# microsoft/KubeGPU

Measured on AMD Instinct MI355X. Metric: scheduled_set_allreduce_busbw_GBps, higher is better.
Workload: dtype uint8; 1 GPU; model=rccl-xgmi-allreduce-probe, global_batch=2000, seq_len=1073741824, parallelism=allreduce-ring-1gpu, mode=hbm_d2d_copy, curve_point=k1-degenerate-hbm, buffer_bytes=1073741824, scenario=BASELINE.json k=1, rank_pinning=ROCR_VISIBLE_DEVICES, pinned_device=0, pinned_bdf=0000:75:00.0, bdf_verified=True

## Files before the change

### kubegpu_amd/csrc/gpuprobe.hip

```cpp

#include <torch/extension.h>
#include <ATen/hip/HIPContext.h>
#include <ATen/hip/impl/HIPGuardImplMasqueradingAsCUDA.h>
#include <hip/hip_runtime.h>

#include <cstdint>

#define WAVE 64
#define BLOCK 256
#define DEFAULT_COPY_BLOCKS 1024
#define DEFAULT_WRITE_BLOCKS 640

__global__ void copy_kernel_v4(const uint4* __restrict__ src,
                               uint4* __restrict__ dst, size_t n4) {
  size_t i = (size_t)blockIdx.x * blockDim.x + threadIdx.x;
  size_t stride = (size_t)gridDim.x * blockDim.x;
  for (; i < n4; i += stride) dst[i] = src[i];
}

typedef unsigned int uint4v __attribute__((ext_vector_type(4)));

__global__ void copy_kernel_v4_nt(const uint4v* __restrict__ src,
                                  uint4v* __restrict__ dst, size_t n4) {
  size_t i = (size_t)blockIdx.x * blockDim.x + threadIdx.x;
  size_t stride = (size_t)gridDim.x * blockDim.x;
  for (; i < n4; i += stride) {
    uint4v v = __builtin_nontemporal_load(&src[i]);
    __builtin_nontemporal_store(v, &dst[i]);
  }
}

__global__ void copy_kernel_v4_nt_u4(const uint4v* __restrict__ src,
                                     uint4v* __restrict__ dst, size_t n4) {
  size_t tid = (size_t)blockIdx.x * blockDim.x + threadIdx.x;
  size_t stride = (size_t)gridDim.x * blockDim.x;
  size_t i = tid;
  size_t bound = n4 >= 3 * stride ? n4 - 3 * stride : 0;
  for (; i < bound; i += 4 * stride) {
    uint4v a = __builtin_nontemporal_load(&src[i]);
    uint4v b = __builtin_nontemporal_load(&src[i + stride]);
    uint4v c = __builtin_nontemporal_load(&src[i + 2 * stride]);
    uint4v d = __builtin_nontemporal_load(&src[i + 3 * stride]);
    __builtin_nontemporal_store(a, &dst[i]);
    __builtin_nontemporal_store(b, &dst[i + stride]);
    __builtin_nontemporal_store(c, &dst[i + 2 * stride]);
    __builtin_nontemporal_store(d, &dst[i + 3 * stride]);
  }
  for (; i < n4; i += stride) {
    uint4v v = __builtin_nontemporal_load(&src[i]);
    __builtin_nontemporal_store(v, &dst[i]);
  }
}

__global__ void copy_kernel_v4_nt_chunk(const uint4v* __restrict__ src,
                                        uint4v* __restrict__ dst, size_t n4) {
  size_t per_block = (n4 + gridDim.x - 1) / gridDim.x;
  size_t begin = (size_t)blockIdx.x * per_block;
  size_t end = begin + per_block < n4 ? begin + per_block : n4;
  for (size_t i = begin + threadIdx.x; i < end; i += blockDim.x) {
    uint4v v = __builtin_nontemporal_load(&src[i]);
    __builtin_nontemporal_store(v, &dst[i]);
  }
}

__global__ void copy_kernel_v4_mixed(const uint4v* __restrict__ src,
                                     uint4v* __restrict__ dst, size_t n4) {
  size_t i = (size_t)blockIdx.x * blockDim.x + threadIdx.x;
  size_t stride = (size_t)gridDim.x * blockDim.x;
  for (; i < n4; i += stride) {
    uint4v v = src[i];
    __builtin_nontemporal_store(v, &dst[i]);
  }
}

__global__ void copy_kernel_b(const unsigned char* __restrict__ src,
                              unsigned char* __restrict__ dst, size_t n) {
  size_t i = (size_t)blockIdx.x * blockDim.x + threadIdx.x;
  size_t stride = (size_t)gridDim.x * blockDim.x;
  for (; i < n; i += stride) dst[i] = src[i];
}

__global__ void read_sum_kernel(const uint4* __restrict__ src, size_t n4,
                                unsigned long long* __restrict__ out) {
  size_t i = (size_t)blockIdx.x * blockDim.x + threadIdx.x;
  size_t stride = (size_t)gridDim.x * blockDim.x;
  unsigned long long acc = 0;
  for (; i < n4; i += stride) {
    uint4 v = src[i];
    acc += (unsigned long long)v.x + v.y + v.z + v.w;
  }
  __shared__ unsigned long long sh[BLOCK / WAVE];
  for (int off = WAVE / 2; off > 0; off >>= 1)
    acc += __shfl_down(acc, off, WAVE);
  int lane = threadIdx.x % WAVE;
  int wid = threadIdx.x / WAVE;
  if (lane == 0) sh[wid] = acc;
  __syncthreads();
  if (threadIdx.x == 0) {
    unsigned long long total = 0;
    for (int w = 0; w < BLOCK / WAVE; ++w) total += sh[w];
    atomicAdd(out, total);
  }
}

__global__ void fill_kernel_v4_nt(uint4v* __restrict__ dst, size_t n4,
                                  unsigned int word) {
  uint4v v = {word, word, word, word};
  size_t i = (size_t)blockIdx.x * blockDim.x + threadIdx.x;
  size_t stride = (size_t)gridDim.x * blockDim.x;
  for (; i < n4; i += stride) __builtin_nontemporal_store(v, &dst[i]);
}


#define MAX_BLOCKS (1 << 20)

static void check_buf(const at::Tensor& t) {
  TORCH_CHECK(t.is_cuda(), "gpuprobe: tensors must be on GPU");
  TORCH_CHECK(t.is_contiguous(), "gpuprobe: tensors must be contiguous");
}

static size_t check_vec_buf(const at::Tensor& t) {
  check_buf(t);
  TORCH_CHECK(t.nbytes() > 0 && t.nbytes() % 16 == 0,
              "gpuprobe: nbytes must be a positive multiple of 16, got ", t.nbytes());
  TORCH_CHECK((uintptr_t)t.data_ptr() % 16 == 0,
              "gpuprobe: tensor storage must be 16-byte aligned");
  return t.nbytes() / 16;
}

static void check_pair(const at::Tensor& dst, const at::Tensor& src) {
  check_buf(dst);
  check_buf(src);
  TORCH_CHECK(src.nbytes() == dst.nbytes(), "gpuprobe: size mismatch");
  TORCH_CHECK(src.device() == dst.device(),
              "gpuprobe: tensors must be on the same device");
  uintptr_t s = (uintptr_t)src.data_ptr(), d = (uintptr_t)dst.data_ptr();
  size_t n = src.nbytes();
  TORCH_CHECK(s == d || s + n <= d || d + n <= s,
              "gpuprobe: dst and src overlap in part");
}

static int check_threads(int64_t threads_arg) {
  TORCH_CHECK(threads_arg >= 0 && threads_arg % WAVE == 0 && threads_arg <= 1024,
              "threads: multiple of 64, <=1024");
  return threads_arg > 0 ? (int)threads_arg : BLOCK;
}

static int pick_blocks(int64_t blocks_arg, size_t n4, int threads, int dflt) {
  TORCH_CHECK(blocks_arg >= 0 && blocks_arg <= MAX_BLOCKS,
              "gpuprobe: blocks out of range 0..", MAX_BLOCKS);
  if (blocks_arg > 0) return (int)blocks_arg;
  return (int)std::min<size_t>((n4 + threads - 1) / threads, (size_t)dflt);
}

static void check_variant(int64_t variant) {
  TORCH_CHECK(variant >= 0 && variant <= 3, "gpuprobe: variant ", variant,
              " out of range 0..3");
}

static void launch_copy(const void* src, void* dst, size_t n4, int64_t variant,
                        bool nontemporal, int blocks, int threads,
                        hipStream_t stream) {
  if (variant == 1)
    hipLaunchKernelGGL(copy_kernel_v4_nt_u4, dim3(blocks), dim3(threads), 0, stream,
                       (const uint4v*)src, (uint4v*)dst, n4);
  else if (variant == 2)
    hipLaunchKernelGGL(copy_kernel_v4_nt_chunk, dim3(blocks), dim3(threads), 0,
                       stream, (const uint4v*)src, (uint4v*)dst, n4);
  else if (variant == 3)
    hipLaunchKernelGGL(copy_kernel_v4_mixed, dim3(blocks), dim3(threads), 0,
                       stream, (const uint4v*)src, (uint4v*)dst, n4);
  else if (nontemporal)
    hipLaunchKernelGGL(copy_kernel_v4_nt, dim3(blocks), dim3(threads), 0, stream,
                       (const uint4v*)src, (uint4v*)dst, n4);
  else
    hipLaunchKernelGGL(copy_kernel_v4, dim3(blocks), dim3(threads), 0, stream,
                       (const uint4*)src, (uint4*)dst, n4);
}

static void launch_read_sum(const void* src, size_t n4, void* out, int blocks,
                            hipStream_t stream) {
  hipLaunchKernelGGL(read_sum_kernel, dim3(blocks), dim3(BLOCK), 0, stream,
                     (const uint4*)src, n4, (unsigned long long*)out);
}

static void launch_fill(void* dst, size_t n4, unsigned int word, int blocks,
                        hipStream_t stream) {
  hipLaunchKernelGGL(fill_kernel_v4_nt, dim3(blocks), dim3(BLOCK), 0, stream,
                     (uint4v*)dst, n4, word);
}

void copy(at::Tensor dst, at::Tensor src) {
  check_pair(dst, src);
  size_t nbytes = src.nbytes();
  if (nbytes == 0) return;
  const at::hip::OptionalHIPGuardMasqueradingAsCUDA guard(at::device_of(dst));
  auto stream = at::hip::getCurrentHIPStream();
  if ((((uintptr_t)src.data_ptr() | (uintptr_t)dst.data_ptr() | nbytes) & 15) == 0) {
    size_t n4 = nbytes / 16;
    int blocks = (int)std::min<size_t>((n4 + BLOCK - 1) / BLOCK, DEFAULT_COPY_BLOCKS);
    launch_copy(src.data_ptr(), dst.data_ptr(), n4, 0, true, blocks, BLOCK, stream);
  } else {
    int blocks = (int)std::min<size_t>((nbytes + BLOCK - 1) / BLOCK, 4096);
    hipLaunchKernelGGL(copy_kernel_b, dim3(blocks), dim3(BLOCK), 0, stream,
                       (const unsigned char*)src.data_ptr(),
                       (unsigned char*)dst.data_ptr(), nbytes);
  }
  C10_HIP_KERNEL_LAUNCH_CHECK();
}

void copy_variant(at::Tensor dst, at::Tensor src, int64_t variant, bool nontemporal,
                  int64_t blocks_arg, int64_t threads_arg) {
  check_pair(dst, src);
  size_t n4 = check_vec_buf(src);
  check_vec_buf(dst);
  check_variant(variant);
  int threads = check_threads(threads_arg);
  int blocks = pick_blocks(blocks_arg, n4, threads, DEFAULT_COPY_BLOCKS);
  const at::hip::OptionalHIPGuardMasqueradingAsCUDA guard(at::device_of(dst));
  auto stream = at::hip::getCurrentHIPStream();
  launch_copy(src.data_ptr(), dst.data_ptr(), n4, variant, nontemporal, blocks,
              threads, stream);
  C10_HIP_KERNEL_LAUNCH_CHECK();
}

uint64_t read_sum(at::Tensor src, int64_t blocks_arg) {
  size_t n4 = check_vec_buf(src);
  int blocks = pick_blocks(blocks_arg, n4, BLOCK, DEFAULT_COPY_BLOCKS);
  const at::hip::OptionalHIPGuardMasqueradingAsCUDA guard(at::device_of(src));
  at::Tensor out = at::zeros({1}, src.options().dtype(at::kLong));
  auto stream = at::hip::getCurrentHIPStream();
  launch_read_sum(src.data_ptr(), n4, out.data_ptr(), blocks, stream);
  C10_HIP_KERNEL_LAUNCH_CHECK();
  C10_HIP_CHECK(hipStreamSynchronize(stream));
  return (uint64_t)out.item<int64_t>();
}

void fill_word(at::Tensor dst, int64_t word, int64_t blocks_arg) {
  size_t n4 = check_vec_buf(dst);
  TORCH_CHECK(word >= 0 && word <= 0xFFFFFFFFLL, "gpuprobe: word must be a u32");
  int blocks = pick_blocks(blocks_arg, n4, BLOCK, DEFAULT_WRITE_BLOCKS);
  const at::hip::OptionalHIPGuardMasqueradingAsCUDA guard(at::device_of(dst));
  auto stream = at::hip::getCurrentHIPStream();
  launch_fill(dst.data_ptr(), n4, (unsigned int)word, blocks, stream);
  C10_HIP_KERNEL_LAUNCH_CHECK();
}

static void check_timed_args(int64_t nbytes, int64_t iters) {
  TORCH_CHECK(nbytes > 0 && nbytes % 16 == 0, "nbytes must be positive, 16-aligned");
  TORCH_CHECK(iters >= 1, "iters must be at least 1");
}

#define POISON 0xA5

template <typename Launch>
static float timed_ms(hipStream_t stream, int64_t iters, Launch&& launch) {
  for (int w = 0; w < 3; ++w) launch();
  hipEvent_t t0, t1;
  (void)hipEventCreate(&t0);
  (void)hipEventCreate(&t1);
  (void)hipEventRecord(t0, stream);
  for (int64_t i = 0; i < iters; ++i) launch();
  (void)hipEventRecord(t1, stream);
  (void)hipEventSynchronize(t1);
  float ms = 0.f;
  (void)hipEventElapsedTime(&ms, t0, t1);
  (void)hipEventDestroy(t0);
  (void)hipEventDestroy(t1);
  C10_HIP_KERNEL_LAUNCH_CHECK();
  return ms;
}

double copy_bw_gbps(int64_t nbytes, int64_t iters, int64_t blocks_arg,
                    bool nontemporal, int64_t variant, int64_t threads_arg) {
  check_timed_args(nbytes, iters);
  check_variant(variant);
  size_t n4 = (size_t)nbytes / 16;
  int threads = check_threads(threads_arg);
  int blocks = pick_blocks(blocks_arg, n4, threads, DEFAULT_COPY_BLOCKS);
  auto opts = at::TensorOptions().dtype(at::kByte).device(at::kCUDA);
  at::Tensor src = at::empty({nbytes}, opts);
  at::Tensor dst = at::empty({nbytes}, opts);
  src.fill_(1);
  dst.fill_(POISON);
  auto stream = at::hip::getCurrentHIPStream();
  float ms = timed_ms(stream, iters, [&]() {
    launch_copy(src.data_ptr(), dst.data_ptr(), n4, variant, nontemporal, blocks,
                threads, stream);
  });
  TORCH_CHECK(at::equal(dst, src), "copy_bw_gbps: variant ", variant,
              " produced wrong output");
  double sec = ms / 1e3;
  return (double)nbytes * 2.0 * iters / sec / 1e9;
}

double write_bw_gbps(int64_t nbytes, int64_t iters, int64_t blocks_arg) {
  check_timed_args(nbytes, iters);
  size_t n4 = (size_t)nbytes / 16;
  int blocks = pick_blocks(blocks_arg, n4, BLOCK, DEFAULT_WRITE_BLOCKS);
  auto opts = at::TensorOptions().dtype(at::kByte).device(at::kCUDA);
  at::Tensor dst = at::empty({nbytes}, opts);
  dst.fill_(POISON);
  auto stream = at::hip::getCurrentHIPStream();
  float ms = timed_ms(stream, iters, [&]() {
    launch_fill(dst.data_ptr(), n4, 0x01010101u, blocks, stream);
  });
  TORCH_CHECK(dst.min().item<uint8_t>() == 1 && dst.max().item<uint8_t>() == 1,
              "write_bw_gbps: fill produced wrong output");
  return (double)nbytes * iters / (ms / 1e3) / 1e9;
}

double read_bw_gbps(int64_t nbytes, int64_t iters, int64_t blocks_arg) {
  check_timed_args(nbytes, iters);
  size_t n4 = (size_t)nbytes / 16;
  int blocks = pick_blocks(blocks_arg, n4, BLOCK, DEFAULT_COPY_BLOCKS);
  auto opts = at::TensorOptions().dtype(at::kByte).device(at::kCUDA);
  at::Tensor src = at::empty({nbytes}, opts);
  src.fill_(1);
  at::Tensor out = at::zeros({1}, at::TensorOptions().dtype(at::kLong).device(at::kCUDA));
  auto stream = at::hip::getCurrentHIPStream();
  float ms = timed_ms(stream, iters, [&]() {
    launch_read_sum(src.data_ptr(), n4, out.data_ptr(), blocks, stream);
  });
  uint64_t want = (uint64_t)(3 + iters) * ((uint64_t)nbytes / 4) * 0x01010101ULL;
  TORCH_CHECK((uint64_t)out.item<int64_t>() == want,
              "read_bw_gbps: read_sum_kernel produced a wrong sum");
  double sec = ms / 1e3;
  return (double)nbytes * iters / sec / 1e9;
}

void bind_memcheck(py::module_& m);
void bind_cucheck(py::module_& m);
void bind_mxcheck(py::module_& m);
void bind_fpcheck(py::module_& m);
void bind_atomcheck(py::module_& m);
void bind_lanecheck(py::module_& m);
void bind_hostlink(py::module_& m);

PYBIND11_MODULE(TORCH_EXTENSION_NAME, m) {
  bind_memcheck(m);
  bind_cucheck(m);
  bind_mxcheck(m);
  bind_fpcheck(m);
  bind_atomcheck(m);
  bind_lanecheck(m);
  bind_hostlink(m);
  m.def("copy", &copy, "streaming uint4 copy kernel (dst, src)",
        py::call_guard<py::gil_scoped_release>());
  m.def("copy_variant", &copy_variant,
        "one untimed launch of a copy_bw_gbps variant (dst, src)",
        py::call_guard<py::gil_scoped_release>(),
        py::arg("dst"), py::arg("src"), py::arg("variant") = 0,
        py::arg("nontemporal") = true, py::arg("blocks") = 0,
        py::arg("threads") = 0);
  m.def("read_sum", &read_sum, "u64 sum of all 32-bit words (one launch)",
        py::call_guard<py::gil_scoped_release>(),
        py::arg("src"), py::arg("blocks") = 0);
  m.def("fill_word", &fill_word, "NT fill of every 32-bit word (one launch)",
        py::call_guard<py::gil_scoped_release>(),
        py::arg("dst"), py::arg("word"), py::arg("blocks") = 0);
  m.def("copy_bw_gbps", &copy_bw_gbps, "timed d2d copy bandwidth",
        py::call_guard<py::gil_scoped_release>(),
        py::arg("nbytes"), py::arg("iters") = 20, py::arg("blocks") = 0,
        py::arg("nontemporal") = true, py::arg("variant") = 0,
        py::arg("threads") = 0);
  m.def("read_bw_gbps", &read_bw_gbps, "timed read bandwidth",
        py::call_guard<py::gil_scoped_release>(),
        py::arg("nbytes"), py::arg("iters") = 20, py::arg("blocks") = 0);
  m.def("write_bw_gbps", &write_bw_gbps, "timed write-only (NT fill) bandwidth",
        py::call_guard<py::gil_scoped_release>(),
        py::arg("nbytes"), py::arg("iters") = 20, py::arg("blocks") = 0);
}
```

### kubegpu_amd/probe/bandwidth.py

```python

from __future__ import annotations

import importlib
import os
import sys

_EXT_DIR = os.path.join(os.path.dirname(os.path.dirname(os.path.abspath(__file__))), "_ext")
_ext = None


class NativeExtensionMissing(RuntimeError):
    pass


def load_ext(required: bool = True):
    global _ext
    if _ext is not None:
        return _ext
    import torch

    if _EXT_DIR not in sys.path:
        sys.path.insert(0, _EXT_DIR)
    try:
        _ext = importlib.import_module("_gpuprobe")
    except ImportError as e:
        if required or torch.cuda.is_available():
            raise NativeExtensionMissing(
                "_gpuprobe HIP extension is not built; run "
                "`python -m kubegpu_amd.build_native` (gfx950) — refusing "
                f"to fall back to eager PyTorch on a GPU box: {e}"
            ) from e
        return None
    return _ext


def copy(dst, src) -> None:
    load_ext().copy(dst, src)


def copy_variant(
    dst,
    src,
    variant: int = 0,
    nontemporal: bool = True,
    blocks: int = 0,
    threads: int = 0,
) -> None:
    load_ext().copy_variant(dst, src, variant, nontemporal, blocks, threads)


def read_sum(src, blocks: int = 0) -> int:
    return load_ext().read_sum(src, blocks)


def fill_word(dst, word: int, blocks: int = 0) -> None:
    load_ext().fill_word(dst, word, blocks)


def d2d_copy_bw_gbps(
    nbytes: int = 1 << 30,
    iters: int = 20,
    blocks: int = 0,
    nontemporal: bool = True,
    variant: int = 0,
) -> float:
    return load_ext().copy_bw_gbps(nbytes, iters, blocks, nontemporal, variant)


def read_bw_gbps(nbytes: int = 1 << 30, iters: int = 20, blocks: int = 0) -> float:
    return load_ext().read_bw_gbps(nbytes, iters, blocks)


def write_bw_gbps(nbytes: int = 1 << 30, iters: int = 20, blocks: int = 0) -> float:
    return load_ext().write_bw_gbps(nbytes, iters, blocks)
```

Before: 5825 GB/s.

## Route aligned copy through unrolled tile kernel with LDS-limited occupancy

Adds a templated tile copy kernel where each block copies contiguous tiles of BLOCK*U vectors with nontemporal loads and stores issued in batches. Occupancy is capped by requesting dummy dynamic LDS so that only a few blocks (three by default) stay resident per CU, and the grid is sized up to MAX_BLOCKS. The default copy() path now uses unroll 2 and residency 3 in place of the grid-stride NT kernel with 1024 blocks. This aims to make DRAM access more address-ordered and cut contention, but fewer resident waves may fail to hide memory latency.

```diff
diff --git a/kubegpu_amd/csrc/gpuprobe.hip b/kubegpu_amd/csrc/gpuprobe.hip
--- a/kubegpu_amd/csrc/gpuprobe.hip
+++ b/kubegpu_amd/csrc/gpuprobe.hip
@@ -4,11 +4,15 @@
 #include <ATen/hip/impl/HIPGuardImplMasqueradingAsCUDA.h>
 #include <hip/hip_runtime.h>
 
+#include <atomic>
 #include <cstdint>
+#include <string>
 
 #define WAVE 64
 #define BLOCK 256
 #define DEFAULT_COPY_BLOCKS 1024
+#define COPY_TILES_UNROLL 2
+#define COPY_TILES_RESIDENT 3
 #define DEFAULT_WRITE_BLOCKS 640
 
 __global__ void copy_kernel_v4(const uint4* __restrict__ src,
@@ -70,6 +74,34 @@
   for (; i < n4; i += stride) {
     uint4v v = src[i];
     __builtin_nontemporal_store(v, &dst[i]);
+  }
+}
+
+template <int U>
+__global__ void __launch_bounds__(BLOCK)
+copy_kernel_tiles(const uint4v* __restrict__ src, uint4v* __restrict__ dst, size_t n4) {
+  constexpr size_t T = (size_t)BLOCK * U;
+  const size_t tiles = (n4 + T - 1) / T;
+  for (size_t t = blockIdx.x; t < tiles; t += gridDim.x) {
+    const size_t base = t * T + threadIdx.x;
+    uint4v v[U];
+    if (t * T + T <= n4) {
+#pragma unroll
+      for (int u = 0; u < U; ++u)
+        v[u] = __builtin_nontemporal_load(&src[base + (size_t)u * BLOCK]);
+#pragma unroll
+      for (int u = 0; u < U; ++u)
+        __builtin_nontemporal_store(v[u], &dst[base + (size_t)u * BLOCK]);
+    } else {
+#pragma unroll
+      for (int u = 0; u < U; ++u)
+        if (base + (size_t)u * BLOCK < n4)
+          v[u] = __builtin_nontemporal_load(&src[base + (size_t)u * BLOCK]);
+#pragma unroll
+      for (int u = 0; u < U; ++u)
+        if (base + (size_t)u * BLOCK < n4)
+          __builtin_nontemporal_store(v[u], &dst[base + (size_t)u * BLOCK]);
+    }
   }
 }
 
@@ -178,6 +210,51 @@
                        (const uint4*)src, (uint4*)dst, n4);
 }
 
+#define CU_LDS_BYTES (160 * 1024)
+#define LDS_GRANULE 1280
+#define MAX_DEVICES 64
+
+static void check_tiles_args(int64_t unroll, int64_t resident, int64_t max_blocks) {
+  TORCH_CHECK(unroll == 1 || unroll == 2 || unroll == 4 || unroll == 8,
+              "gpuprobe: unroll must be 1, 2, 4 or 8, got ", unroll);
+  TORCH_CHECK(resident >= 0 && resident <= 8, "gpuprobe: resident ", resident,
+              " out of range 0..8");
+  TORCH_CHECK(max_blocks >= 0 && max_blocks <= MAX_BLOCKS,
+              "gpuprobe: max_blocks out of range 0..", MAX_BLOCKS);
+}
+
+template <int U>
+static void launch_copy_tiles_u(const void* src, void* dst, size_t n4, int resident,
+                                int max_blocks, hipStream_t stream) {
+  size_t tiles = (n4 + (size_t)BLOCK * U - 1) / ((size_t)BLOCK * U);
+  size_t cap = max_blocks > 0 ? (size_t)max_blocks : (size_t)MAX_BLOCKS;
+  size_t lds = resident > 0 ? CU_LDS_BYTES / resident / LDS_GRANULE * LDS_GRANULE : 0;
+  if (lds > 64 * 1024) {
+    static std::atomic<bool> raised[MAX_DEVICES];
+    int dev = 0;
+    C10_HIP_CHECK(hipGetDevice(&dev));
+    TORCH_CHECK(dev >= 0 && dev < MAX_DEVICES, "gpuprobe: device index ", dev);
+    if (!raised[dev].load(std::memory_order_acquire)) {
+      C10_HIP_CHECK(hipFuncSetAttribute((const void*)copy_kernel_tiles<U>,
+                                        hipFuncAttributeMaxDynamicSharedMemorySize,
+                                        CU_LDS_BYTES));
+      raised[dev].store(true, std::memory_order_release);
+    }
+  }
+  hipLaunchKernelGGL(copy_kernel_tiles<U>, dim3((unsigned)std::min(tiles, cap)),
+                     dim3(BLOCK), lds, stream, (const uint4v*)src, (uint4v*)dst, n4);
+}
+
+static void launch_copy_tiles(const void* src, void* dst, size_t n4, int unroll,
+                              int resident, int max_blocks, hipStream_t stream) {
+  switch (unroll) {
+    case 1: launch_copy_tiles_u<1>(src, dst, n4, resident, max_blocks, stream); break;
+    case 2: launch_copy_tiles_u<2>(src, dst, n4, resident, max_blocks, stream); break;
+    case 4: launch_copy_tiles_u<4>(src, dst, n4, resident, max_blocks, stream); break;
+    default: launch_copy_tiles_u<8>(src, dst, n4, resident, max_blocks, stream); break;
+  }
+}
+
 static void launch_read_sum(const void* src, size_t n4, void* out, int blocks,
                             hipStream_t stream) {
   hipLaunchKernelGGL(read_sum_kernel, dim3(blocks), dim3(BLOCK), 0, stream,
@@ -197,9 +274,8 @@
   const at::hip::OptionalHIPGuardMasqueradingAsCUDA guard(at::device_of(dst));
   auto stream = at::hip::getCurrentHIPStream();
   if ((((uintptr_t)src.data_ptr() | (uintptr_t)dst.data_ptr() | nbytes) & 15) == 0) {
-    size_t n4 = nbytes / 16;
-    int blocks = (int)std::min<size_t>((n4 + BLOCK - 1) / BLOCK, DEFAULT_COPY_BLOCKS);
-    launch_copy(src.data_ptr(), dst.data_ptr(), n4, 0, true, blocks, BLOCK, stream);
+    launch_copy_tiles(src.data_ptr(), dst.data_ptr(), nbytes / 16, COPY_TILES_UNROLL,
+                      COPY_TILES_RESIDENT, 0, stream);
   } else {
     int blocks = (int)std::min<size_t>((nbytes + BLOCK - 1) / BLOCK, 4096);
     hipLaunchKernelGGL(copy_kernel_b, dim3(blocks), dim3(BLOCK), 0, stream,
@@ -221,6 +297,19 @@
   auto stream = at::hip::getCurrentHIPStream();
   launch_copy(src.data_ptr(), dst.data_ptr(), n4, variant, nontemporal, blocks,
               threads, stream);
+  C10_HIP_KERNEL_LAUNCH_CHECK();
+}
+
+void copy_tiles(at::Tensor dst, at::Tensor src, int64_t unroll, int64_t resident,
+                int64_t max_blocks) {
+  check_pair(dst, src);
+  size_t n4 = check_vec_buf(src);
+  check_vec_buf(dst);
+  check_tiles_args(unroll, resident, max_blocks);
+  const at::hip::OptionalHIPGuardMasqueradingAsCUDA guard(at::device_of(dst));
+  auto stream = at::hip::getCurrentHIPStream();
+  launch_copy_tiles(src.data_ptr(), dst.data_ptr(), n4, (int)unroll, (int)resident,
+                    (int)max_blocks, stream);
   C10_HIP_KERNEL_LAUNCH_CHECK();
 }
 
@@ -271,6 +360,22 @@
   return ms;
 }
 
+template <typename Launch>
+static double timed_copy_gbps(int64_t nbytes, int64_t iters, const std::string& who,
+                              Launch&& launch) {
+  auto opts = at::TensorOptions().dtype(at::kByte).device(at::kCUDA);
+  at::Tensor src = at::empty({nbytes}, opts);
+  at::Tensor dst = at::empty({nbytes}, opts);
+  src.fill_(1);
+  dst.fill_(POISON);
+  auto stream = at::hip::getCurrentHIPStream();
+  float ms = timed_ms(stream, iters,
+                      [&]() { launch(src.data_ptr(), dst.data_ptr(), stream); });
+  TORCH_CHECK(at::equal(dst, src), who, " produced wrong output");
+  double sec = ms / 1e3;
+  return (double)nbytes * 2.0 * iters / sec / 1e9;
+}
+
 double copy_bw_gbps(int64_t nbytes, int64_t iters, int64_t blocks_arg,
                     bool nontemporal, int64_t variant, int64_t threads_arg) {
   check_timed_args(nbytes, iters);
@@ -278,20 +383,21 @@
   size_t n4 = (size_t)nbytes / 16;
   int threads = check_threads(threads_arg);
   int blocks = pick_blocks(blocks_arg, n4, threads, DEFAULT_COPY_BLOCKS);
-  auto opts = at::TensorOptions().dtype(at::kByte).device(at::kCUDA);
-  at::Tensor src = at::empty({nbytes}, opts);
-  at::Tensor dst = at::empty({nbytes}, opts);
-  src.fill_(1);
-  dst.fill_(POISON);
-  auto stream = at::hip::getCurrentHIPStream();
-  float ms = timed_ms(stream, iters, [&]() {
-    launch_copy(src.data_ptr(), dst.data_ptr(), n4, variant, nontemporal, blocks,
-                threads, stream);
+  return timed_copy_gbps(nbytes, iters, "copy_bw_gbps: variant " + std::to_string(variant),
+                         [&](const void* src, void* dst, hipStream_t stream) {
+    launch_copy(src, dst, n4, variant, nontemporal, blocks, threads, stream);
   });
-  TORCH_CHECK(at::equal(dst, src), "copy_bw_gbps: variant ", variant,
-              " produced wrong output");
-  double sec = ms / 1e3;
-  return (double)nbytes * 2.0 * iters / sec / 1e9;
+}
+
+double copy_tiles_bw_gbps(int64_t nbytes, int64_t iters, int64_t unroll,
+                          int64_t resident, int64_t max_blocks) {
+  check_timed_args(nbytes, iters);
+  check_tiles_args(unroll, resident, max_blocks);
+  size_t n4 = (size_t)nbytes / 16;
+  return timed_copy_gbps(nbytes, iters, "copy_tiles_bw_gbps: the tile kernel",
+                         [&](const void* src, void* dst, hipStream_t stream) {
+    launch_copy_tiles(src, dst, n4, (int)unroll, (int)resident, (int)max_blocks, stream);
+  });
 }
 
 double write_bw_gbps(int64_t nbytes, int64_t iters, int64_t blocks_arg) {
@@ -353,6 +459,16 @@
         py::arg("dst"), py::arg("src"), py::arg("variant") = 0,
         py::arg("nontemporal") = true, py::arg("blocks") = 0,
         py::arg("threads") = 0);
+  m.def("copy_tiles", &copy_tiles,
+        "one untimed launch of the address-ordered tile copy kernel (dst, src)",
+        py::call_guard<py::gil_scoped_release>(),
+        py::arg("dst"), py::arg("src"), py::arg("unroll"), py::arg("resident"),
+        py::arg("max_blocks") = 0);
+  m.def("copy_tiles_bw_gbps", &copy_tiles_bw_gbps,
+        "timed d2d copy bandwidth of the tile copy kernel",
+        py::call_guard<py::gil_scoped_release>(),
+        py::arg("nbytes"), py::arg("iters"), py::arg("unroll"), py::arg("resident"),
+        py::arg("max_blocks") = 0);
   m.def("read_sum", &read_sum, "u64 sum of all 32-bit words (one launch)",
         py::call_guard<py::gil_scoped_release>(),
         py::arg("src"), py::arg("blocks") = 0);
diff --git a/kubegpu_amd/probe/bandwidth.py b/kubegpu_amd/probe/bandwidth.py
--- a/kubegpu_amd/probe/bandwidth.py
+++ b/kubegpu_amd/probe/bandwidth.py
@@ -49,6 +49,10 @@
     load_ext().copy_variant(dst, src, variant, nontemporal, blocks, threads)
 
 
+def copy_tiles(dst, src, unroll: int, resident: int, max_blocks: int = 0) -> None:
+    load_ext().copy_tiles(dst, src, unroll, resident, max_blocks)
+
+
 def read_sum(src, blocks: int = 0) -> int:
     return load_ext().read_sum(src, blocks)
 
@@ -67,6 +71,16 @@
     return load_ext().copy_bw_gbps(nbytes, iters, blocks, nontemporal, variant)
 
 
+def d2d_copy_tiles_bw_gbps(
+    nbytes: int = 1 << 30,
+    iters: int = 20,
+    unroll: int = 1,
+    resident: int = 0,
+    max_blocks: int = 0,
+) -> float:
+    return load_ext().copy_tiles_bw_gbps(nbytes, iters, unroll, resident, max_blocks)
+
+
 def read_bw_gbps(nbytes: int = 1 << 30, iters: int = 20, blocks: int = 0) -> float:
     return load_ext().read_bw_gbps(nbytes, iters, blocks)
 
```

Result: faster. 6675 GB/s (median of 6 runs) (+14.6%).
